# kobigurk/phase2-bn254

Measured on AMD Instinct MI355X. Metric: BN254 G1 MSM throughput (Mscalar-mul/s) at 2^26 points, higher is better.
Workload: dtype u32x8 (256-bit Montgomery limbs)

## Files before the change

### phase2-bn254_amd/csrc/msm_common.hpp

```cpp
#pragma once
#include <stdint.h>

namespace zk {

constexpr uint32_t SIGN_BIT = 0x80000000u;

struct MsmGeom {
  uint32_t c;
  uint32_t W;
  uint32_t nb;
  uint8_t width[64];
  uint8_t shift[64];
  uint32_t rmul;
  uint32_t rshift;
};

constexpr uint32_t MSM_SIZE_BINS = 4096;
constexpr uint32_t PART_THREADS = 1024;
constexpr uint32_t PART_MAX_ST = 16384;
constexpr uint32_t PART_MAX_EB = PART_MAX_ST / PART_THREADS;
constexpr uint32_t PART_LO_MAX = 12;
constexpr uint32_t PART_EC = 32;
constexpr uint32_t PART_LDS_A = 76 * 1024;
constexpr uint32_t PART_LDS_MAX = 160 * 1024 - 512;
constexpr uint32_t KEY_NONE_MASK = 0x00ffffffu;

struct PartGeom {
  uint32_t lo_bits;
  uint32_t nbin;
  uint32_t st;
  uint32_t n_st;
  uint32_t n_chunk;
  uint32_t rows_per_chunk;
};

constexpr uint32_t BIG_SEG = PART_EC * PART_THREADS;

struct BigPlan {
  uint32_t n_big;
  uint32_t total_seg;
};

constexpr uint32_t MSM_HEAVY_BLOCKS = 65536;
constexpr uint32_t MSM_HEAVY_SEG = 4096;
constexpr uint32_t MSM_HEAVY_LANES = 64;
constexpr uint32_t MSM_PAIR_MAX_BUCKETS = 3u << 17;

constexpr uint32_t MSM_FINAL_MAX = 1024;
constexpr uint32_t MSM_TREE_SLICE = 512;
// ... 5 lines not shown
```

### phase2-bn254_amd/csrc/msm_partition.hip

```cpp
#include "msm_partition.hpp"

#include <map>
#include <mutex>
#include <vector>

#include "field.hpp"
#include "msm_digits.hpp"

namespace zk {

std::atomic<int> g_msm_inflight[16];

namespace {


template <class In, class Out>
__device__ __forceinline__ uint32_t block_scan_1024(uint32_t len, uint32_t* scratch, In value, Out out) {
  constexpr uint32_t PER = 4;
  const uint32_t tid = threadIdx.x, lane = tid & 63u, wv = tid >> 6;
  uint32_t v[PER], sum = 0;
#pragma unroll
  for (uint32_t k = 0; k < PER; ++k) {
    const uint32_t idx = tid * PER + k;
    v[k] = idx < len ? value(idx) : 0u;
// ... 80 lines not shown
        for (int l = 0; l < 8; ++l) s[l] = f.l[l];
      }
      const uint32_t any = s[0] | s[1] | s[2] | s[3] | s[4] | s[5] | s[6] | s[7];
      if (active && (s[7] >> 30)) {
        atomicMin(err_scalar, (unsigned long long)(i + i_bias));
        active = false;
      }
      if (!active || any == 0) {
        for (uint32_t wl = 0; wl < WL; ++wl) keys[(uint64_t)wl * kstride + i] = G.nb;
        continue;
      }
      msm_scalar_digits<RM>(s, G, w_lo, w_hi < G.W ? w_hi : G.W, [&](uint32_t w, uint32_t d, uint32_t neg) {
        if (w >= w_lo && w < w_hi) {
          const uint32_t wl = w - w_lo;
          keys[(uint64_t)wl * kstride + i] = d ? ((d - 1) | neg) : G.nb;
          if (d) {
            const uint32_t cell = wl * P.nbin + ((d - 1) >> P.lo_bits);
            atomicAdd(&lh[cell >> 1], 1u << (16u * (cell & 1u)));
          }
        }
      });
    }
    __syncthreads();
    uint32_t* row = reinterpret_cast<uint32_t*>(tile_hist) + (uint64_t)st * nword;
    for (uint32_t t = threadIdx.x; t < nword; t += PART_THREADS) row[t] = lh[t];
    __syncthreads();
  }
}

template <uint32_t RM>
__global__ void __launch_bounds__(256) msm_digits_plain_kernel(const uint32_t* __restrict__ scalars, uint64_t n, const uint32_t* __restrict__ density,
                                                              MsmGeom G, uint32_t w_lo, uint32_t w_hi, int scalars_mont, uint64_t kstride,
// ... 31 lines not shown
  msm_scalar_digits<RM>(s, G, w_lo, w_hi < G.W ? w_hi : G.W, [&](uint32_t w, uint32_t d, uint32_t neg) {
    if (w >= w_lo && w < w_hi) keys[(uint64_t)(w - w_lo) * kstride + i] = d ? ((d - 1) | neg) : G.nb;
  });
}

__global__ void __launch_bounds__(PART_THREADS) msm_tile_hist_kernel(const uint32_t* __restrict__ keys, uint64_t n, uint64_t kstride, uint32_t nb,
                                                                     uint32_t WL, PartGeom P, uint16_t* __restrict__ tile_hist) {
  extern __shared__ __attribute__((aligned(16))) unsigned char smem[];
  uint32_t* lh = reinterpret_cast<uint32_t*>(smem);
  const uint32_t st = blockIdx.x % P.n_st, wl = blockIdx.x / P.n_st;
  const uint64_t i0 = (uint64_t)st * P.st;
  const uint32_t cnt = (uint32_t)(n - i0 < P.st ? n - i0 : P.st);
  for (uint32_t t = threadIdx.x; t < P.nbin; t += PART_THREADS) lh[t] = 0;
  __syncthreads();
  const uint32_t* kp = keys + (uint64_t)wl * kstride + i0;
  for (uint32_t idx = 4u * threadIdx.x; idx < cnt; idx += 4u * PART_THREADS) {
    uint32_t v[4] = {nb, nb, nb, nb};
    if (idx + 4 <= cnt) {
      const uint4 q = *reinterpret_cast<const uint4*>(kp + idx);
      v[0] = q.x; v[1] = q.y; v[2] = q.z; v[3] = q.w;
    } else {
      for (uint32_t e = 0; e < 4; ++e)
        if (idx + e < cnt) v[e] = kp[idx + e];
    }
#pragma unroll
    for (uint32_t e = 0; e < 4; ++e) {
      const uint32_t b = v[e] & KEY_NONE_MASK;
      if (b < nb) atomicAdd(&lh[b >> P.lo_bits], 1u);
    }
  }
  __syncthreads();
  const uint32_t ncell = WL * P.nbin, stride = (ncell + 1u) & ~1u;
  uint16_t* row = tile_hist + (uint64_t)st * stride + (uint64_t)wl * P.nbin;
  for (uint32_t t = threadIdx.x; t < P.nbin; t += PART_THREADS) row[t] = (uint16_t)lh[t];
}

__global__ void __launch_bounds__(256) msm_colsum_kernel(const uint16_t* __restrict__ tile_hist, PartGeom P, uint32_t ncell,
                                                        uint32_t* __restrict__ csum) {
  const uint32_t col = blockIdx.x * blockDim.x + threadIdx.x, chunk = blockIdx.y;
  if (col >= ncell) return;
  const uint32_t stride = (ncell + 1u) & ~1u;
  const uint32_t r0 = chunk * P.rows_per_chunk, r1 = r0 + P.rows_per_chunk < P.n_st ? r0 + P.rows_per_chunk : P.n_st;
  uint32_t s = 0;
#pragma unroll 8
  for (uint32_t r = r0; r < r1; ++r) s += tile_hist[(uint64_t)r * stride + col];
// ... 3 lines not shown
__global__ void __launch_bounds__(256) msm_colscan_kernel(uint32_t* __restrict__ csum, PartGeom P, uint32_t ncell, uint32_t* __restrict__ total) {
  const uint32_t col = blockIdx.x * blockDim.x + threadIdx.x;
  if (col >= ncell) return;
  uint32_t run = 0;
  for (uint32_t ch = 0; ch < P.n_chunk; ++ch) {
    const uint32_t v = csum[(uint64_t)ch * ncell + col];
    csum[(uint64_t)ch * ncell + col] = run;
    run += v;
  }
  total[col] = run;
}

__global__ void __launch_bounds__(PART_THREADS) msm_binscan_kernel(const uint32_t* __restrict__ total, PartGeom P, uint32_t ncell, uint32_t nb,
                                                                   uint32_t* __restrict__ bin_start, uint32_t* __restrict__ out_start) {
  __shared__ uint32_t scratch[32];
  auto padded = [&](uint32_t col) {
    const uint32_t bin = col % P.nbin;
    const uint32_t nf = ((bin + 1) << P.lo_bits) <= nb ? 1u << P.lo_bits : nb - (bin << P.lo_bits);
    return (total[col] + 3u * nf + 3u) & ~3u;
  };
  const uint32_t t0 = block_scan_long(ncell, scratch, [&](uint32_t c) { return total[c]; }, [&](uint32_t c, uint32_t ex) { bin_start[c] = ex; });
  const uint32_t t1 = block_scan_long(ncell, scratch, padded, [&](uint32_t c, uint32_t ex) { out_start[c] = ex; });
  if (threadIdx.x == 0) {
    bin_start[ncell] = t0;
    out_start[ncell] = t1;
  }
}

__global__ void __launch_bounds__(256) msm_tileoff_kernel(const uint16_t* __restrict__ tile_hist, const uint32_t* __restrict__ cbase,
                                                         const uint32_t* __restrict__ bin_start, PartGeom P, uint32_t ncell,
                                                         uint32_t* __restrict__ tile_off) {
  const uint32_t col = blockIdx.x * blockDim.x + threadIdx.x, chunk = blockIdx.y;
  if (col >= ncell) return;
  const uint32_t stride = (ncell + 1u) & ~1u;
  const uint32_t r0 = chunk * P.rows_per_chunk, r1 = r0 + P.rows_per_chunk < P.n_st ? r0 + P.rows_per_chunk : P.n_st;
// ... 23 lines not shown
    const uint32_t b = blockIdx.x;
    if (per != 0 && b < body * WL) {
      const uint32_t x = b % xcds, j = b / xcds;
      st = x * per + j % per;
      wl = j / per;
    } else {
      const uint32_t r = b - body * WL, rem = P.n_st - body;
      st = body + r % rem;
      wl = r / rem;
    }
  }
  const uint64_t i0 = (uint64_t)st * P.st;
  const uint32_t cnt = (uint32_t)(n - i0 < P.st ? n - i0 : P.st);
  for (uint32_t t = threadIdx.x; t < P.nbin; t += PART_THREADS) loff[t] = 0;
  __syncthreads();
  uint32_t key[PART_MAX_EB], rank[PART_MAX_EB];
  const uint32_t* kp = keys + (uint64_t)wl * kstride + i0;
  const bool wide = true;
#pragma unroll
  for (uint32_t k4 = 0; k4 < PART_MAX_EB / 4; ++k4) {
    const uint32_t idx = 4u * (k4 * PART_THREADS + threadIdx.x);
    uint32_t v[4] = {nb, nb, nb, nb};
    if (wide && idx + 4 <= cnt) {
      const uint4 q = *reinterpret_cast<const uint4*>(kp + idx);
      v[0] = q.x; v[1] = q.y; v[2] = q.z; v[3] = q.w;
    } else {
#pragma unroll
      for (uint32_t e = 0; e < 4; ++e)
        if (idx + e < cnt) v[e] = kp[idx + e];
    }
#pragma unroll
    for (uint32_t e = 0; e < 4; ++e) {
      key[4 * k4 + e] = v[e];
      rank[4 * k4 + e] = 0;
      const uint32_t b = v[e] & KEY_NONE_MASK;
      if (b < nb) rank[4 * k4 + e] = atomicAdd(&loff[b >> P.lo_bits], 1u);
    }
  }
  __syncthreads();
  const uint32_t* toff = tile_off + ((uint64_t)st * WL + wl) * P.nbin;
  const uint32_t total = block_scan_1024(P.nbin, scratch, [&](uint32_t x) { return loff[x]; },
                                         [&](uint32_t x, uint32_t ex) { loff[x] = ex; delta[x] = toff[x] - ex; });
  __syncthreads();
#pragma unroll
  for (uint32_t k4 = 0; k4 < PART_MAX_EB / 4; ++k4) {
#pragma unroll
    for (uint32_t e = 0; e < 4; ++e) {
      const uint32_t k = 4 * k4 + e;
      const uint32_t idx = 4u * (k4 * PART_THREADS + threadIdx.x) + e;
      const uint32_t b = key[k] & KEY_NONE_MASK;
      if (idx < cnt && b < nb) {
        uint64_t i = i0 + idx, tw = 0;
        if (flat_stride != 0) {
          tw = i / flat_stride;
          i -= tw * flat_stride;
          tw *= table_stride;
        }
        uint64_t bi = base_offset + i;
        if (density != nullptr) {
          const uint32_t wd = density[i >> 5];
          bi = base_offset + dprefix[i >> 5] + __popc(wd & ((1u << (i & 31)) - 1u));
        }
        bi += tw;
        staging[loff[b >> P.lo_bits] + rank[k]] = make_uint2(key[k], (uint32_t)bi);
      }
    }
  }
  __syncthreads();
  for (uint32_t p = threadIdx.x; p < total; p += PART_THREADS) {
    const uint2 e = staging[p];
    pairs[(uint64_t)(p + delta[(e.x & KEY_NONE_MASK) >> P.lo_bits])] = e;
  }
}

__global__ void __launch_bounds__(PART_THREADS) msm_bucket_kernel(const uint2* __restrict__ pairs, const uint32_t* __restrict__ bin_start,
                                                                  const uint32_t* __restrict__ out_start, uint32_t nb, PartGeom P,
                                                                  uint32_t stage_cap, uint32_t* __restrict__ first, uint32_t* __restrict__ last,
                                                                  uint32_t* __restrict__ vals) {
  extern __shared__ __attribute__((aligned(16))) unsigned char smem[];
  const uint32_t nfmax = 1u << P.lo_bits;
  const uint32_t nfl = nfmax < 4 ? 4 : nfmax;
  uint32_t* hist = reinterpret_cast<uint32_t*>(smem);
  uint32_t* start = hist + nfl;
  uint32_t* scratch = start + nfl;
  uint32_t* staging = scratch + 32;
  const uint32_t col = blockIdx.x, wl = col / P.nbin, bin = col % P.nbin;
  const uint32_t beg = bin_start[col], cnt = bin_start[col + 1] - beg;
  const uint32_t ob = out_start[col];
  const uint32_t nf = (bin + 1) << P.lo_bits <= nb ? nfmax : nb - (bin << P.lo_bits);
  const uint32_t fmask = nfmax - 1u;
  for (uint32_t t = threadIdx.x; t < nfmax; t += PART_THREADS) hist[t] = 0;
  __syncthreads();
  if (cnt > PART_EC * PART_THREADS) return;
  uint32_t val[PART_EC], fr[PART_EC];
#pragma unroll
  for (uint32_t k = 0; k < PART_EC; ++k) {
    const uint32_t idx = k * PART_THREADS + threadIdx.x;
    val[k] = 0;
    fr[k] = 0;
    if (idx < cnt) {
      const uint2 e = pairs[(uint64_t)beg + idx];
      const uint32_t f = e.x & fmask;
      val[k] = e.y | (e.x & SIGN_BIT);
      fr[k] = f | (atomicAdd(&hist[f], 1u) << PART_LO_MAX);
    }
  }
  __syncthreads();
  const uint32_t padded = block_scan_1024(nf, scratch, [&](uint32_t x) { return (hist[x] + 3u) & ~3u; },
                                          [&](uint32_t x, uint32_t ex) { start[x] = ex; });
  __syncthreads();
  const uint32_t id0 = wl * nb + (bin << P.lo_bits);
  for (uint32_t t = threadIdx.x; t < nf; t += PART_THREADS) {
    first[id0 + t] = ob + start[t];
    last[id0 + t] = ob + start[t] + hist[t];
  }
  if (padded <= stage_cap) {
#pragma unroll
    for (uint32_t k = 0; k < PART_EC; ++k) {
      const uint32_t idx = k * PART_THREADS + threadIdx.x;
      if (idx < cnt) staging[start[fr[k] & ((1u << PART_LO_MAX) - 1u)] + (fr[k] >> PART_LO_MAX)] = val[k];
    }
    __syncthreads();
    uint4* dst = reinterpret_cast<uint4*>(vals + ob);
    const uint4* src = reinterpret_cast<const uint4*>(staging);
    for (uint32_t q = threadIdx.x; q < padded / 4; q += PART_THREADS) dst[q] = src[q];
  } else {
// ... 24 lines not shown

__global__ void __launch_bounds__(PART_THREADS) msm_scan_small_kernel(const uint16_t* __restrict__ tile_hist, PartGeom P, uint32_t ncell, uint32_t nb,
                                                                      uint32_t* __restrict__ col_total, uint32_t* __restrict__ bin_start,
                                                                      uint32_t* __restrict__ out_start, uint32_t* __restrict__ tile_off,
                                                                      uint32_t* __restrict__ size_hist, uint32_t* __restrict__ big_col,
                                                                      uint32_t* __restrict__ big_seg_off, BigPlan* __restrict__ plan) {
  __shared__ uint32_t scratch[32];
  const uint32_t stride = (ncell + 1u) & ~1u;
  for (uint32_t t = threadIdx.x; t < MSM_SIZE_BINS; t += PART_THREADS) size_hist[t] = 0;
  for (uint32_t col = threadIdx.x; col < ncell; col += PART_THREADS) {
    uint32_t s = 0;
    for (uint32_t r = 0; r < P.n_st; ++r) s += tile_hist[(uint64_t)r * stride + col];
    col_total[col] = s;
  }
  __syncthreads();
  auto padded = [&](uint32_t col) {
    const uint32_t bin = col % P.nbin;
    const uint32_t nf = ((bin + 1) << P.lo_bits) <= nb ? 1u << P.lo_bits : nb - (bin << P.lo_bits);
    return (col_total[col] + 3u * nf + 3u) & ~3u;
  };
  const uint32_t t0 = block_scan_long(ncell, scratch, [&](uint32_t c) { return col_total[c]; }, [&](uint32_t c, uint32_t ex) { bin_start[c] = ex; });
  const uint32_t t1 = block_scan_long(ncell, scratch, padded, [&](uint32_t c, uint32_t ex) { out_start[c] = ex; });
  if (threadIdx.x == 0) {
    bin_start[ncell] = t0;
    out_start[ncell] = t1;
  }
  __syncthreads();
  for (uint32_t col = threadIdx.x; col < ncell; col += PART_THREADS) {
    uint32_t run = bin_start[col];
    for (uint32_t r = 0; r < P.n_st; ++r) {
      tile_off[(uint64_t)r * ncell + col] = run;
      run += tile_hist[(uint64_t)r * stride + col];
    }
  }
  auto cnt_of = [&](uint32_t col) { return bin_start[col + 1] - bin_start[col]; };
// ... 19 lines not shown
  }
  *col = big_col[lo];
  *seg = b - big_seg_off[lo];
  return true;
}

__global__ void __launch_bounds__(PART_THREADS) msm_bigbin_count_kernel(const uint2* __restrict__ pairs, const uint32_t* __restrict__ bin_start,
                                                                        const BigPlan* __restrict__ plan, const uint32_t* __restrict__ big_col,
                                                                        const uint32_t* __restrict__ big_seg_off, uint32_t nb, PartGeom P,
                                                                        uint32_t* __restrict__ gcnt) {
  extern __shared__ __attribute__((aligned(16))) unsigned char smem[];
  uint32_t* hist = reinterpret_cast<uint32_t*>(smem);
  for (uint32_t b = blockIdx.x;; b += gridDim.x) {
    uint32_t col, seg;
    if (!bigbin_locate(plan, big_col, big_seg_off, b, &col, &seg)) return;
    const uint32_t nfmax = 1u << P.lo_bits, fmask = nfmax - 1u;
    const uint32_t wl = col / P.nbin, bin = col % P.nbin;
    const uint32_t beg = bin_start[col] + seg * BIG_SEG, end = bin_start[col + 1];
    const uint32_t cnt = end - beg < BIG_SEG ? end - beg : BIG_SEG;
    for (uint32_t t = threadIdx.x; t < nfmax; t += PART_THREADS) hist[t] = 0;
    __syncthreads();
    for (uint32_t idx = threadIdx.x; idx < cnt; idx += PART_THREADS) atomicAdd(&hist[pairs[(uint64_t)beg + idx].x & fmask], 1u);
    __syncthreads();
    const uint32_t id0 = wl * nb + (bin << P.lo_bits);
    for (uint32_t t = threadIdx.x; t < nfmax; t += PART_THREADS)
      if (hist[t]) atomicAdd(&gcnt[id0 + t], hist[t]);
    __syncthreads();
  }
}

__global__ void __launch_bounds__(PART_THREADS) msm_bigbin_place_kernel(const uint2* __restrict__ pairs, const uint32_t* __restrict__ bin_start,
                                                                        const uint32_t* __restrict__ out_start, const BigPlan* __restrict__ plan,
                                                                        const uint32_t* __restrict__ big_col, const uint32_t* __restrict__ big_seg_off,
                                                                        uint32_t nb, PartGeom P, int staged, const uint32_t* __restrict__ gcnt,
                                                                        uint32_t* __restrict__ gcur, uint32_t* __restrict__ first,
                                                                        uint32_t* __restrict__ last, uint32_t* __restrict__ vals) {
  extern __shared__ __attribute__((aligned(16))) unsigned char smem[];
  for (uint32_t blk = blockIdx.x;; blk += gridDim.x) {
  uint32_t col, seg;
  if (!bigbin_locate(plan, big_col, big_seg_off, blk, &col, &seg)) return;
  const uint32_t nfmax = 1u << P.lo_bits, fmask = nfmax - 1u;
  const uint32_t nfl = nfmax < 4 ? 4 : nfmax;
  uint32_t* hist = reinterpret_cast<uint32_t*>(smem);
  uint32_t* start = hist + nfl;
  uint32_t* scratch = start + nfl;
  uint32_t* lstart = scratch + 32;
  uint32_t* llen = lstart + nfl;
  uint32_t* staging = llen + nfl;
  const uint32_t wl = col / P.nbin, bin = col % P.nbin;
  const uint32_t beg = bin_start[col] + seg * BIG_SEG, end = bin_start[col + 1];
  const uint32_t cnt = end - beg < BIG_SEG ? end - beg : BIG_SEG;
  const uint32_t ob = out_start[col];
  const uint32_t nf = (bin + 1) << P.lo_bits <= nb ? nfmax : nb - (bin << P.lo_bits);
  const uint32_t id0 = wl * nb + (bin << P.lo_bits);
  for (uint32_t t = threadIdx.x; t < nfmax; t += PART_THREADS) hist[t] = 0;
  __syncthreads();
  uint32_t val[PART_EC], fr[PART_EC];
#pragma unroll
  for (uint32_t k = 0; k < PART_EC; ++k) {
    const uint32_t idx = k * PART_THREADS + threadIdx.x;
    val[k] = 0;
    fr[k] = 0;
    if (idx < cnt) {
      const uint2 e = pairs[(uint64_t)beg + idx];
      const uint32_t f = e.x & fmask;
      val[k] = e.y | (e.x & SIGN_BIT);
      fr[k] = f | (atomicAdd(&hist[f], 1u) << PART_LO_MAX);
    }
  }
  __syncthreads();
  block_scan_1024(nf, scratch, [&](uint32_t x) { return (gcnt[id0 + x] + 3u) & ~3u; }, [&](uint32_t x, uint32_t ex) { start[x] = ex; });
  if (staged) block_scan_1024(nf, scratch, [&](uint32_t x) { return hist[x]; }, [&](uint32_t x, uint32_t ex) { lstart[x] = ex; });
  __syncthreads();
  for (uint32_t t = threadIdx.x; t < nf; t += PART_THREADS) {
    if (seg == 0) {
      first[id0 + t] = ob + start[t];
      last[id0 + t] = ob + start[t] + gcnt[id0 + t];
    }
    const uint32_t mine = hist[t];
    if (staged) llen[t] = mine;
// ... 136 lines not shown
  for (const void* fn : fns) {
    hipError_t e = hipFuncSetAttribute(fn, hipFuncAttributeMaxDynamicSharedMemorySize, 160 * 1024);
    if (e != hipSuccess) {
      std::fprintf(stderr, "[mi355zk] hipFuncSetAttribute(partition kernel, 160 KiB LDS) failed: %s\n", hipGetErrorString(e));
      rc = ZK_ERR_DEVICE;
    }
  }
  g_part_cfg[dev] = rc;
  return rc;
}

int msm_checkpoint(const MsmPartCall& A, const char* what, const ChunkPlan& C) {
  if (!A.knobs.debug) return 0;
  const MsmPlan& P = A.plan;
  ZK_HIP(hipStreamSynchronize(A.st));
  std::fprintf(stderr, "[mi355zk] msm<%d> n=%llu chunk@%llu+%llu c=%u W=%u buckets=%u levels=%u part(lo=%u nbin=%u st=%u): %s done\n", A.group,
               (unsigned long long)A.n, (unsigned long long)C.lo, (unsigned long long)C.n, P.G.c, P.WL, P.n_buckets, P.n_levels, C.P.lo_bits, C.P.nbin,
               C.P.st, what);
  return 0;
}

void msm_order_by_size(const uint32_t* first, const uint32_t* last, uint32_t n_buckets, uint32_t* hist, uint32_t* order, uint32_t* sizes_sorted,
                       hipStream_t st) {
  uint32_t hb = (n_buckets + 4095) / 4096;
  hipLaunchKernelGGL(msm_size_hist_kernel, dim3(hb < 1024 ? hb : 1024), dim3(1024), 0, st, first, last, n_buckets, hist);
  hipLaunchKernelGGL(msm_size_scan_kernel, dim3(1), dim3(1024), 0, st, hist);
  hipLaunchKernelGGL(msm_size_scatter_kernel, dim3((n_buckets + 1024 * MSM_SCATTER_PER - 1) / (1024 * MSM_SCATTER_PER)), dim3(1024), 0, st, first,
                     last, n_buckets, hist, order, sizes_sorted);
}

void launch_heavy_plan(hipStream_t st, const uint32_t* sizes_sorted, uint32_t hb, uint32_t heavy, uint32_t seg, uint32_t* item_off) {
  hipLaunchKernelGGL(msm_heavy_plan_kernel, dim3(1), dim3(1024), 0, st, sizes_sorted, hb, heavy, seg, item_off);
}
// ... 56 lines not shown
    hipLaunchKernelGGL(msm_tileoff_kernel, dim3((ncell + 255) / 256, PG.n_chunk), dim3(256), 0, st, W.tile_hist, W.csum, W.bin_start, PG, ncell, W.tile_off);
  }
  ZK_HIP(hipGetLastError());
  prof_end(S.scan, st);
  prof_begin(S.scatter, st);
  hipLaunchKernelGGL(msm_scatter_kernel, dim3(PG.n_st * WL), dim3(PART_THREADS), (size_t)(2 * ((PG.nbin + 3u) & ~3u) + 32) * 4 + (size_t)PG.st * 8, st,
                     W.keys, C.np, P.tmode ? C.np : kstride, boff, dens, dpre, G.nb, WL, PG, A.knobs.part_xcds, W.tile_off, W.pairs, P.tmode ? kstride : 0ull,
                     A.table_stride);
  ZK_HIP(hipGetLastError());
  prof_end(S.scatter, st);
  if (msm_checkpoint(A, "scatter", C)) return ZK_ERR_DEVICE;
  prof_begin(S.bucket, st);
  {
    const uint32_t nfl = (1u << PG.lo_bits) < 4 ? 4 : (1u << PG.lo_bits);
    const size_t fixed = (size_t)(2 * nfl + 32) * 4;
    uint64_t want = (uint64_t)(C.np / PG.nbin) * 5 / 4 + 3ull * nfl + 4096;
    const uint64_t cap_max = (PART_LDS_MAX - fixed) / 4;
    if (want > cap_max) want = cap_max;
    if (want > (uint64_t)PART_EC * PART_THREADS + 3ull * nfl) want = (uint64_t)PART_EC * PART_THREADS + 3ull * nfl;
    const uint32_t stage_cap = (uint32_t)want & ~3u;
    hipLaunchKernelGGL(msm_bucket_kernel, dim3(ncell), dim3(PART_THREADS), fixed + (size_t)stage_cap * 4, st, W.pairs, W.bin_start, W.out_start, G.nb, PG,
                       stage_cap, W.first, W.last, W.vals_b);
    if (C.np > BIG_SEG) {
      const uint32_t max_seg = (uint32_t)(2 * (C.m / BIG_SEG) + 2);
      if (!C.small_scan) hipLaunchKernelGGL(msm_bigbin_plan_kernel, dim3(1), dim3(PART_THREADS), 0, st, W.bin_start, ncell, W.big_col, W.big_seg, W.big_plan);
      int n_cu = 256;
      (void)hipDeviceGetAttribute(&n_cu, hipDeviceAttributeMultiprocessorCount, A.dev);
      const uint32_t big_grid = max_seg < 2u * (uint32_t)n_cu ? max_seg : 2u * (uint32_t)n_cu;
      const uint32_t place_grid = max_seg < (uint32_t)n_cu ? max_seg : (uint32_t)n_cu;
      hipLaunchKernelGGL(msm_bigbin_count_kernel, dim3(big_grid), dim3(PART_THREADS), (size_t)nfl * 4, st, W.pairs, W.bin_start, W.big_plan, W.big_col, W.big_seg,
                         G.nb, PG, W.gcnt);
// ... 52 lines not shown
```

### phase2-bn254_amd/csrc/msm_plan.hpp

```cpp
#pragma once
#include <algorithm>
#include <cmath>
#include <cstdio>
#include <cstdlib>
#include <vector>

#include "host_util.hpp"
#include "msm_common.hpp"

namespace zk {

struct MsmKnobs {
  int msm_c = 0;
  uint32_t radix_m = 0, radix_s = 0;
  bool radix_off = false;
  int table_c = 0;
  int part_lo = -1, part_st = 0;
  bool no_tail2d = false;
  bool no_small_scan = false;
  bool debug = false;
  bool fused_a = false;
  uint32_t part_xcds = 8;
  bool acc_a4 = true;
  int g1_pair = -1, g2_pair = -1;
// ... 83 lines not shown

inline MsmGeom make_geom_radix(uint32_t rmul, uint32_t rshift) {
  MsmGeom G{};
  G.rmul = rmul;
  G.rshift = rshift;
  const double B = std::ldexp((double)rmul, (int)rshift);
  G.nb = (rmul << rshift) / 2;
  G.c = 1;
  while ((1u << G.c) <= G.nb) ++G.c;
  uint32_t W = 2;
  while ((W - 1) * std::log2(B) + std::log2((double)G.nb) < 254.001) ++W;
  G.W = W;
  return G;
}

inline double geom_cost(double W, double nbk, double field_bits, uint64_t n, double top_values) {
  double cost = W * ((10.0 + 0.7 * std::ceil(field_bits / 8.0)) * (double)n + 45.0 * nbk);
  double lanes = W * nbk;
  if (lanes < 131072.0) cost *= (1.0 + 0.5 * (131072.0 / lanes - 1.0));
  const double mean = (double)n / nbk;
  const double heavy = std::max(64.0, 2.0 * mean + 16.0);
  const double top_len = (double)n / top_values;
  if (top_len > heavy) cost += 1.2e7;
  else if (top_len > 2.0 * mean + 16.0) cost += (top_len - (2.0 * mean + 16.0)) * 5e5;
  return cost;
}

inline MsmGeom choose_geom(uint64_t n, int group, uint32_t wgroups, const MsmKnobs& K) {
  if (K.radix_m && wgroups == 1) return make_geom_radix(K.radix_m, K.radix_s);
  if (K.msm_c >= 2 && K.msm_c <= 24 && wgroups == 1) return make_geom((uint32_t)K.msm_c);
  if (wgroups == 1 && n < (1ull << 20)) {
    uint32_t lg = 0;
    while ((1ull << lg) < n) ++lg;
    uint32_t c = lg <= 10 ? 10u : lg <= 12 ? 11u : lg == 13 ? 12u : lg <= 15 ? 13u : lg <= 17 ? 15u : 16u;
    if (group == 2) c = lg <= 10 ? 10u : lg == 11 ? 11u : lg <= 15 ? 12u : lg <= 17 ? 14u : lg == 18 ? 15u : 16u;
    return make_geom(c);
  }
  uint32_t best_c = 0;
  double best = 1e300;
  for (uint32_t c = 4; c <= 24; ++c) {
    double W = std::ceil((254.0 + 1.0) / c);
    if ((uint32_t)W % wgroups) continue;
    const MsmGeom Gc = make_geom(c);
    double cost = geom_cost(W, std::ldexp(1.0, (int)c - 1), c, n, std::ldexp(1.0, (int)Gc.width[Gc.W - 1]));
    if (cost < best) { best = cost; best_c = c; }
  }
  MsmGeom G{};
  if (best_c) G = make_geom(best_c);
  if (K.radix_off && best_c) return G;
  for (uint32_t rmul = 3; rmul <= 15; rmul += 2)
    for (uint32_t rshift = 4; rshift <= 22; ++rshift) {
      MsmGeom R = make_geom_radix(rmul, rshift);
      if (R.W > 64 || R.c > 24 || R.W % wgroups) continue;
      const double top_values = std::exp2(254.0 - (R.W - 1.0) * std::log2(std::ldexp((double)rmul, (int)rshift)));
      double cost = geom_cost(R.W, R.nb, R.c, n, top_values);
      if (cost < 0.985 * best) { best = cost / 0.985; G = R; }
    }
  return G;
}

inline uint32_t table_window_bits(uint64_t n_bases, int group, const MsmKnobs& K) {
  if (K.table_c >= 4 && K.table_c <= 24) return (uint32_t)K.table_c;
  uint32_t lg = 0;
  while ((1ull << lg) < n_bases) ++lg;
  if (group == 2) return lg <= 18 ? 17u : lg == 19 ? 19u : 20u;
  return lg <= 16 ? 17u : lg <= 22 ? 20u : 22u;
}

inline PartGeom choose_part(uint64_t n, uint32_t WL, uint32_t nb, const MsmKnobs& K) {
  PartGeom P{};
  uint32_t lo_cap = 0;
  while ((1u << lo_cap) < nb && lo_cap < PART_LO_MAX) ++lo_cap;
  auto nbin_of = [&](uint32_t lo) { return (uint32_t)(((uint64_t)nb + (1ull << lo) - 1) >> lo); };
  auto fits_lds = [&](uint32_t lo, uint64_t budget) { return (uint64_t)WL * nbin_of(lo) * 2 <= budget && nbin_of(lo) <= 4 * PART_THREADS; };
  auto fits = [&](uint32_t lo) { return fits_lds(lo, 2 * PART_LDS_A); };
  auto pop = [&](uint32_t lo) { return (uint64_t)n * (1ull << lo) / nb; };
  uint32_t lo = lo_cap;
  const uint64_t pop_target = 12288;
  const uint64_t pop_cap = (uint64_t)PART_EC * PART_THREADS * 85 / 100;
  while (lo > 0 && pop(lo) > pop_target && fits_lds(lo - 1, PART_LDS_A)) --lo;
  while (lo > 0 && pop(lo) > pop_cap && fits(lo - 1)) --lo;
  while (!fits(lo) && lo < PART_LO_MAX) ++lo;
  if (K.part_lo >= 0 && K.part_lo <= (int)lo_cap && fits((uint32_t)K.part_lo)) lo = (uint32_t)K.part_lo;
  P.lo_bits = lo;
  P.nbin = nbin_of(lo);
  uint32_t st = PART_MAX_ST;
  while (st > PART_THREADS && (n / st) * WL < 256) st >>= 1;
  if (K.part_st >= (int)PART_THREADS && K.part_st <= (int)PART_MAX_ST && K.part_st % (int)PART_THREADS == 0) st = (uint32_t)K.part_st;
  while (st > PART_THREADS && (uint64_t)st * 8 + (uint64_t)P.nbin * 8 + 256 > PART_LDS_MAX) st -= PART_THREADS;
  if ((uint64_t)st * 8 + (uint64_t)P.nbin * 8 + 256 > PART_LDS_MAX) st = 0;
  P.st = st;
  P.n_st = (uint32_t)((n + st - 1) / st);
  P.rows_per_chunk = P.n_st > 64 ? (P.n_st + 63) / 64 : 1;
  P.n_chunk = (P.n_st + P.rows_per_chunk - 1) / P.rows_per_chunk;
  return P;
}


struct MsmRequest {
  int group = 1;
  uint64_t n = 0;
  uint64_t base_offset = 0;
  uint32_t wgroups = 1, wgroup = 0;
  uint32_t n_chunks = 1;
  const uint64_t* cuts = nullptr;
  bool two_sets = false;
  uint64_t table_stride = 0;
  uint32_t table_c = 0;
};

struct ChunkPlan {
  uint64_t lo, n, m, np;
  PartGeom P;
  uint32_t ncell, heavy, heavy_seg, hb, max_items;
  bool small_scan;
  uint32_t split_t, split_hb;
};

struct MsmLayout {
  size_t keys, pairs, tile_hist, tile_off, csum, total, bin_start, out_start;
  size_t gcnt, gcur, big_col, big_seg, big_plan;
  size_t first, last, hist, sizes_b, ids_b, item_off, seg_sums, buckets, partA, partS;
  size_t rc;
  size_t wsums;
  size_t err;
  size_t sumtmp;
  size_t total_bytes;
  size_t back_bytes() const { return (err - wsums) + 16; }
};
// ... 34 lines not shown
  const uint32_t n_chunks = R.n_chunks;
  const uint64_t* cuts = R.cuts ? R.cuts : whole;
  if (n_chunks == 0 || (R.cuts == nullptr && n_chunks != 1) || cuts[0] != 0 || cuts[n_chunks] != n) return ZK_ERR_BAD_ARGS;
  if (n_chunks > 1 && R.two_sets) return ZK_ERR_BAD_ARGS;
  uint64_t n_max = 0;
  for (uint32_t c = 0; c < n_chunks; ++c) {
    if (cuts[c + 1] <= cuts[c] || (c > 0 && (cuts[c] & 31))) return ZK_ERR_BAD_ARGS;
    if (cuts[c + 1] - cuts[c] > n_max) n_max = cuts[c + 1] - cuts[c];
  }
  const MsmGeom G = P.G = tmode ? make_geom(R.table_c) : choose_geom(n, R.group, R.wgroups, K);
  if (G.W == 0 || G.W % R.wgroups) return ZK_ERR_BAD_ARGS;
  const uint32_t WD = P.WD = G.W / R.wgroups;
  P.w_lo = R.wgroup * WD;
  P.w_hi = P.w_lo + WD;
  const uint32_t WL = P.WL = tmode ? 1u : WD;
  if (tmode && (uint64_t)G.W * R.table_stride > 0x7fffffffull) return ZK_ERR_BAD_ARGS;
  const uint64_t m_max = P.m_max = tmode ? ((n_max + 3) & ~3ull) * WD : n_max * WL;
  if (m_max > 0xfffffff0ull) return ZK_ERR_BAD_ARGS;
  const uint32_t n_buckets = P.n_buckets = WL * G.nb;
  uint32_t final_cnt = G.nb, n_levels = 0;
  auto tail_fits = [&](uint32_t cnt) { return !K.no_tail2d && g1 && (uint64_t)cnt * WL <= (1ull << 17) && cnt >= (1u << 15) && cnt <= (1u << 18); };
  while (final_cnt > K.final_max && n_levels < MSM_MAX_LEVELS) {
    if (tail_fits(final_cnt)) break;
    uint32_t logl = (uint64_t)final_cnt * WL >= (1ull << 20) ? 3 : 2;
    if (K.logl[n_levels]) logl = K.logl[n_levels];
    P.lvl_cnt[n_levels] = final_cnt;
    P.lvl_logl[n_levels] = logl;
    P.lvl_chunks[n_levels] = (final_cnt + (1u << logl) - 1) >> logl;
    P.total_chunks += P.lvl_chunks[n_levels];
    final_cnt = P.lvl_chunks[n_levels];
// ... 9 lines not shown
    P.cols_log = (lg + 1) / 2;
  }
  const uint32_t t_cols = P.t_cols = tail2d ? 1u << P.cols_log : final_cnt, t_rows = P.t_rows = tail2d ? (final_cnt + t_cols - 1) / t_cols : 0;
  while ((1u << P.final_bits) <= t_cols - 1 + final_off) ++P.final_bits;
  while (t_rows > 1 && (1u << P.row_bits) <= t_rows - 1) ++P.row_bits;

  P.chunks.resize(n_chunks);
  uint64_t keys_cap = 0, tile_hist_b = 0, tile_off_b = 0, csum_b = 0;
  uint32_t ncell_max = 0, hb_max = 0, items_max = 0;
  for (uint32_t c = 0; c < n_chunks; ++c) {
    ChunkPlan& C = P.chunks[c];
    C.lo = cuts[c];
    C.n = cuts[c + 1] - cuts[c];
    C.np = tmode ? ((C.n + 3) & ~3ull) * WD : C.n;
    C.m = C.np * WL;
    C.P = choose_part(C.np, WL, G.nb, K);
    if (C.P.st == 0) return ZK_ERR_BAD_ARGS;
    C.ncell = WL * C.P.nbin;
    C.small_scan = !K.no_small_scan && (uint64_t)C.P.n_st * C.ncell <= (1u << 16);
    const uint64_t vals_cap = C.m + 3ull * n_buckets + 4ull * C.ncell + 4;
    if (vals_cap > 0xfffffff0ull) return ZK_ERR_BAD_ARGS;
    keys_cap = std::max(keys_cap, vals_cap);
    tile_hist_b = std::max<uint64_t>(tile_hist_b, (uint64_t)C.P.n_st * ((C.ncell + 1) & ~1u) * 2);
    tile_off_b = std::max<uint64_t>(tile_off_b, (uint64_t)C.P.n_st * C.ncell * 4);
    csum_b = std::max<uint64_t>(csum_b, (uint64_t)C.P.n_chunk * C.ncell * 4);
    ncell_max = std::max(ncell_max, C.ncell);
    const uint64_t mean_len = C.m / n_buckets + 1;
    uint64_t heavy64 = mean_len * 8 + 1024;
    const uint64_t heavy_cap = (C.m >> 17) > 64 ? (C.m >> 17) : 64;
    if (heavy64 > heavy_cap) heavy64 = heavy_cap;
    if (heavy64 < 2 * mean_len + 16) heavy64 = 2 * mean_len + 16;
    C.heavy = (uint32_t)(heavy64 > 0xffffffffull ? 0xffffffffull : heavy64);
    C.heavy_seg = 128;
// ... 65 lines not shown
```

Measured before the change: 1011.

## Use finer partition bins for the sparsely populated top window

The top MSM window holds only a small range of digit values, so with uniform coarse bins its points pile into a few overloaded bins. The change adds per-window bin widths (a split point and a smaller lo width) for the last window, so its populated range spreads over more bins. Digits above the reachable range are skipped, and their bucket first/last entries are zeroed directly. This targets load imbalance and oversized bins in the partition and bucket kernels, at the cost of extra index arithmetic per key and a larger PartGeom kernel argument.

Result: no change. 1012 (median of 2 runs) (+0.1%).

```diff
diff --git a/phase2-bn254_amd/csrc/msm_common.hpp b/phase2-bn254_amd/csrc/msm_common.hpp
--- a/phase2-bn254_amd/csrc/msm_common.hpp
+++ b/phase2-bn254_amd/csrc/msm_common.hpp
@@ -25,6 +25,8 @@
 constexpr uint32_t PART_LDS_MAX = 160 * 1024 - 512;
 constexpr uint32_t KEY_NONE_MASK = 0x00ffffffu;
 
+constexpr uint32_t PART_MAX_W = 72;
+
 struct PartGeom {
   uint32_t lo_bits;
   uint32_t nbin;
@@ -32,7 +34,27 @@
   uint32_t n_st;
   uint32_t n_chunk;
   uint32_t rows_per_chunk;
+  uint16_t split_w[PART_MAX_W];
+  uint8_t lo_w[PART_MAX_W];
+
+  constexpr uint32_t edge(uint32_t wl) const { return (uint32_t)split_w[wl] << lo_w[wl]; }
+  constexpr uint32_t part_end(uint32_t wl, uint32_t nb) const {
+    const uint64_t e = (uint64_t)edge(wl) + ((uint64_t)(nbin - split_w[wl]) << lo_bits);
+    return e < nb ? (uint32_t)e : nb;
+  }
 };
+
+constexpr uint32_t part_bin_of(uint32_t b, uint32_t lo_w, uint32_t split, uint32_t lo_bits) {
+  const uint32_t edge = split << lo_w;
+  return b < edge ? b >> lo_w : split + ((b - edge) >> lo_bits);
+}
+struct PartCell { uint32_t wl, base, bits, count; };
+constexpr PartCell part_cell(const PartGeom& P, uint32_t col, uint32_t nb) {
+  const uint32_t wl = col / P.nbin, bin = col % P.nbin, lo_w = P.lo_w[wl], split = P.split_w[wl];
+  const uint32_t base = bin < split ? bin << lo_w : (split << lo_w) + ((bin - split) << P.lo_bits), bits = bin < split ? lo_w : P.lo_bits;
+  const uint32_t end = P.part_end(wl, nb);
+  return {wl, base, bits, base >= end ? 0u : end - base < (1u << bits) ? end - base : 1u << bits};
+}
 
 constexpr uint32_t BIG_SEG = PART_EC * PART_THREADS;
 
diff --git a/phase2-bn254_amd/csrc/msm_partition.hip b/phase2-bn254_amd/csrc/msm_partition.hip
--- a/phase2-bn254_amd/csrc/msm_partition.hip
+++ b/phase2-bn254_amd/csrc/msm_partition.hip
@@ -118,8 +118,8 @@
         if (w >= w_lo && w < w_hi) {
           const uint32_t wl = w - w_lo;
           keys[(uint64_t)wl * kstride + i] = d ? ((d - 1) | neg) : G.nb;
-          if (d) {
-            const uint32_t cell = wl * P.nbin + ((d - 1) >> P.lo_bits);
+          if (d && d - 1 < P.part_end(wl, G.nb)) {
+            const uint32_t cell = wl * P.nbin + part_bin_of(d - 1, P.lo_w[wl], P.split_w[wl], P.lo_bits);
             atomicAdd(&lh[cell >> 1], 1u << (16u * (cell & 1u)));
           }
         }
@@ -181,21 +181,26 @@
   for (uint32_t t = threadIdx.x; t < P.nbin; t += PART_THREADS) lh[t] = 0;
   __syncthreads();
   const uint32_t* kp = keys + (uint64_t)wl * kstride + i0;
-  for (uint32_t idx = 4u * threadIdx.x; idx < cnt; idx += 4u * PART_THREADS) {
-    uint32_t v[4] = {nb, nb, nb, nb};
-    if (idx + 4 <= cnt) {
-      const uint4 q = *reinterpret_cast<const uint4*>(kp + idx);
-      v[0] = q.x; v[1] = q.y; v[2] = q.z; v[3] = q.w;
-    } else {
-      for (uint32_t e = 0; e < 4; ++e)
-        if (idx + e < cnt) v[e] = kp[idx + e];
-    }
-#pragma unroll
-    for (uint32_t e = 0; e < 4; ++e) {
-      const uint32_t b = v[e] & KEY_NONE_MASK;
-      if (b < nb) atomicAdd(&lh[b >> P.lo_bits], 1u);
-    }
-  }
+  const uint32_t lo_w = P.lo_w[wl], split = P.split_w[wl], end = P.part_end(wl, nb);
+  auto count = [&](auto bin_of) {
+    for (uint32_t idx = 4u * threadIdx.x; idx < cnt; idx += 4u * PART_THREADS) {
+      uint32_t v[4] = {nb, nb, nb, nb};
+      if (idx + 4 <= cnt) {
+        const uint4 q = *reinterpret_cast<const uint4*>(kp + idx);
+        v[0] = q.x; v[1] = q.y; v[2] = q.z; v[3] = q.w;
+      } else {
+        for (uint32_t e = 0; e < 4; ++e)
+          if (idx + e < cnt) v[e] = kp[idx + e];
+      }
+#pragma unroll
+      for (uint32_t e = 0; e < 4; ++e) {
+        const uint32_t b = v[e] & KEY_NONE_MASK;
+        if (b < end) atomicAdd(&lh[bin_of(b)], 1u);
+      }
+    }
+  };
+  if (lo_w == P.lo_bits) count([&](uint32_t b) { return b >> P.lo_bits; });
+  else count([&](uint32_t b) { return part_bin_of(b, lo_w, split, P.lo_bits); });
   __syncthreads();
   const uint32_t ncell = WL * P.nbin, stride = (ncell + 1u) & ~1u;
   uint16_t* row = tile_hist + (uint64_t)st * stride + (uint64_t)wl * P.nbin;
@@ -229,11 +234,7 @@
 __global__ void __launch_bounds__(PART_THREADS) msm_binscan_kernel(const uint32_t* __restrict__ total, PartGeom P, uint32_t ncell, uint32_t nb,
                                                                    uint32_t* __restrict__ bin_start, uint32_t* __restrict__ out_start) {
   __shared__ uint32_t scratch[32];
-  auto padded = [&](uint32_t col) {
-    const uint32_t bin = col % P.nbin;
-    const uint32_t nf = ((bin + 1) << P.lo_bits) <= nb ? 1u << P.lo_bits : nb - (bin << P.lo_bits);
-    return (total[col] + 3u * nf + 3u) & ~3u;
-  };
+  auto padded = [&](uint32_t col) { return (total[col] + 3u * part_cell(P, col, nb).count + 3u) & ~3u; };
   const uint32_t t0 = block_scan_long(ncell, scratch, [&](uint32_t c) { return total[c]; }, [&](uint32_t c, uint32_t ex) { bin_start[c] = ex; });
   const uint32_t t1 = block_scan_long(ncell, scratch, padded, [&](uint32_t c, uint32_t ex) { out_start[c] = ex; });
   if (threadIdx.x == 0) {
@@ -287,63 +288,68 @@
   const uint32_t cnt = (uint32_t)(n - i0 < P.st ? n - i0 : P.st);
   for (uint32_t t = threadIdx.x; t < P.nbin; t += PART_THREADS) loff[t] = 0;
   __syncthreads();
-  uint32_t key[PART_MAX_EB], rank[PART_MAX_EB];
   const uint32_t* kp = keys + (uint64_t)wl * kstride + i0;
-  const bool wide = true;
-#pragma unroll
-  for (uint32_t k4 = 0; k4 < PART_MAX_EB / 4; ++k4) {
-    const uint32_t idx = 4u * (k4 * PART_THREADS + threadIdx.x);
-    uint32_t v[4] = {nb, nb, nb, nb};
-    if (wide && idx + 4 <= cnt) {
-      const uint4 q = *reinterpret_cast<const uint4*>(kp + idx);
-      v[0] = q.x; v[1] = q.y; v[2] = q.z; v[3] = q.w;
-    } else {
-#pragma unroll
-      for (uint32_t e = 0; e < 4; ++e)
-        if (idx + e < cnt) v[e] = kp[idx + e];
-    }
-#pragma unroll
-    for (uint32_t e = 0; e < 4; ++e) {
-      key[4 * k4 + e] = v[e];
-      rank[4 * k4 + e] = 0;
-      const uint32_t b = v[e] & KEY_NONE_MASK;
-      if (b < nb) rank[4 * k4 + e] = atomicAdd(&loff[b >> P.lo_bits], 1u);
-    }
-  }
-  __syncthreads();
-  const uint32_t* toff = tile_off + ((uint64_t)st * WL + wl) * P.nbin;
-  const uint32_t total = block_scan_1024(P.nbin, scratch, [&](uint32_t x) { return loff[x]; },
-                                         [&](uint32_t x, uint32_t ex) { loff[x] = ex; delta[x] = toff[x] - ex; });
-  __syncthreads();
-#pragma unroll
-  for (uint32_t k4 = 0; k4 < PART_MAX_EB / 4; ++k4) {
-#pragma unroll
-    for (uint32_t e = 0; e < 4; ++e) {
-      const uint32_t k = 4 * k4 + e;
-      const uint32_t idx = 4u * (k4 * PART_THREADS + threadIdx.x) + e;
-      const uint32_t b = key[k] & KEY_NONE_MASK;
-      if (idx < cnt && b < nb) {
-        uint64_t i = i0 + idx, tw = 0;
-        if (flat_stride != 0) {
-          tw = i / flat_stride;
-          i -= tw * flat_stride;
-          tw *= table_stride;
+  const uint32_t lo_w = P.lo_w[wl], split = P.split_w[wl], end = P.part_end(wl, nb);
+  auto run = [&](auto bin_of) {
+    uint32_t key[PART_MAX_EB], rank[PART_MAX_EB];
+    const bool wide = true;
+#pragma unroll
+    for (uint32_t k4 = 0; k4 < PART_MAX_EB / 4; ++k4) {
+      const uint32_t idx = 4u * (k4 * PART_THREADS + threadIdx.x);
+      uint32_t v[4] = {nb, nb, nb, nb};
+      if (wide && idx + 4 <= cnt) {
+        const uint4 q = *reinterpret_cast<const uint4*>(kp + idx);
+        v[0] = q.x; v[1] = q.y; v[2] = q.z; v[3] = q.w;
+      } else {
+#pragma unroll
+        for (uint32_t e = 0; e < 4; ++e)
+          if (idx + e < cnt) v[e] = kp[idx + e];
+      }
+#pragma unroll
+      for (uint32_t e = 0; e < 4; ++e) {
+        key[4 * k4 + e] = v[e];
+        rank[4 * k4 + e] = 0;
+        const uint32_t b = v[e] & KEY_NONE_MASK;
+        if (b < end) rank[4 * k4 + e] = atomicAdd(&loff[bin_of(b)], 1u);
+      }
+    }
+    __syncthreads();
+    const uint32_t* toff = tile_off + ((uint64_t)st * WL + wl) * P.nbin;
+    const uint32_t total = block_scan_1024(P.nbin, scratch, [&](uint32_t x) { return loff[x]; },
+                                           [&](uint32_t x, uint32_t ex) { loff[x] = ex; delta[x] = toff[x] - ex; });
+    __syncthreads();
+#pragma unroll
+    for (uint32_t k4 = 0; k4 < PART_MAX_EB / 4; ++k4) {
+#pragma unroll
+      for (uint32_t e = 0; e < 4; ++e) {
+        const uint32_t k = 4 * k4 + e;
+        const uint32_t idx = 4u * (k4 * PART_THREADS + threadIdx.x) + e;
+        const uint32_t b = key[k] & KEY_NONE_MASK;
+        if (idx < cnt && b < end) {
+          uint64_t i = i0 + idx, tw = 0;
+          if (flat_stride != 0) {
+            tw = i / flat_stride;
+            i -= tw * flat_stride;
+            tw *= table_stride;
+          }
+          uint64_t bi = base_offset + i;
+          if (density != nullptr) {
+            const uint32_t wd = density[i >> 5];
+            bi = base_offset + dprefix[i >> 5] + __popc(wd & ((1u << (i & 31)) - 1u));
+          }
+          bi += tw;
+          staging[loff[bin_of(b)] + rank[k]] = make_uint2(key[k], (uint32_t)bi);
         }
-        uint64_t bi = base_offset + i;
-        if (density != nullptr) {
-          const uint32_t wd = density[i >> 5];
-          bi = base_offset + dprefix[i >> 5] + __popc(wd & ((1u << (i & 31)) - 1u));
-        }
-        bi += tw;
-        staging[loff[b >> P.lo_bits] + rank[k]] = make_uint2(key[k], (uint32_t)bi);
-      }
-    }
-  }
-  __syncthreads();
-  for (uint32_t p = threadIdx.x; p < total; p += PART_THREADS) {
-    const uint2 e = staging[p];
-    pairs[(uint64_t)(p + delta[(e.x & KEY_NONE_MASK) >> P.lo_bits])] = e;
-  }
+      }
+    }
+    __syncthreads();
+    for (uint32_t p = threadIdx.x; p < total; p += PART_THREADS) {
+      const uint2 e = staging[p];
+      pairs[(uint64_t)(p + delta[bin_of(e.x & KEY_NONE_MASK)])] = e;
+    }
+  };
+  if (lo_w == P.lo_bits) run([&](uint32_t b) { return b >> P.lo_bits; });
+  else run([&](uint32_t b) { return part_bin_of(b, lo_w, split, P.lo_bits); });
 }
 
 __global__ void __launch_bounds__(PART_THREADS) msm_bucket_kernel(const uint2* __restrict__ pairs, const uint32_t* __restrict__ bin_start,
@@ -351,18 +357,22 @@
                                                                   uint32_t stage_cap, uint32_t* __restrict__ first, uint32_t* __restrict__ last,
                                                                   uint32_t* __restrict__ vals) {
   extern __shared__ __attribute__((aligned(16))) unsigned char smem[];
-  const uint32_t nfmax = 1u << P.lo_bits;
-  const uint32_t nfl = nfmax < 4 ? 4 : nfmax;
+  const uint32_t nfl = (1u << P.lo_bits) < 4 ? 4 : 1u << P.lo_bits;
   uint32_t* hist = reinterpret_cast<uint32_t*>(smem);
   uint32_t* start = hist + nfl;
   uint32_t* scratch = start + nfl;
   uint32_t* staging = scratch + 32;
-  const uint32_t col = blockIdx.x, wl = col / P.nbin, bin = col % P.nbin;
+  const uint32_t col = blockIdx.x;
+  const PartCell cell = part_cell(P, col, nb);
+  const uint32_t wl = cell.wl, nf = cell.count;
   const uint32_t beg = bin_start[col], cnt = bin_start[col + 1] - beg;
   const uint32_t ob = out_start[col];
-  const uint32_t nf = (bin + 1) << P.lo_bits <= nb ? nfmax : nb - (bin << P.lo_bits);
-  const uint32_t fmask = nfmax - 1u;
-  for (uint32_t t = threadIdx.x; t < nfmax; t += PART_THREADS) hist[t] = 0;
+  const uint32_t end = P.part_end(wl, nb);
+  if (end < nb) {
+    const uint32_t per = (nb - end + P.nbin - 1) / P.nbin, t0 = end + (col % P.nbin) * per;
+    for (uint32_t t = t0 + threadIdx.x; t < t0 + per && t < nb; t += PART_THREADS) first[wl * nb + t] = last[wl * nb + t] = 0;
+  }
+  for (uint32_t t = threadIdx.x; t < nf; t += PART_THREADS) hist[t] = 0;
   __syncthreads();
   if (cnt > PART_EC * PART_THREADS) return;
   uint32_t val[PART_EC], fr[PART_EC];
@@ -373,7 +383,7 @@
     fr[k] = 0;
     if (idx < cnt) {
       const uint2 e = pairs[(uint64_t)beg + idx];
-      const uint32_t f = e.x & fmask;
+      const uint32_t f = (e.x & KEY_NONE_MASK) - cell.base;
       val[k] = e.y | (e.x & SIGN_BIT);
       fr[k] = f | (atomicAdd(&hist[f], 1u) << PART_LO_MAX);
     }
@@ -382,7 +392,7 @@
   const uint32_t padded = block_scan_1024(nf, scratch, [&](uint32_t x) { return (hist[x] + 3u) & ~3u; },
                                           [&](uint32_t x, uint32_t ex) { start[x] = ex; });
   __syncthreads();
-  const uint32_t id0 = wl * nb + (bin << P.lo_bits);
+  const uint32_t id0 = wl * nb + cell.base;
   for (uint32_t t = threadIdx.x; t < nf; t += PART_THREADS) {
     first[id0 + t] = ob + start[t];
     last[id0 + t] = ob + start[t] + hist[t];
@@ -437,11 +447,7 @@
     col_total[col] = s;
   }
   __syncthreads();
-  auto padded = [&](uint32_t col) {
-    const uint32_t bin = col % P.nbin;
-    const uint32_t nf = ((bin + 1) << P.lo_bits) <= nb ? 1u << P.lo_bits : nb - (bin << P.lo_bits);
-    return (col_total[col] + 3u * nf + 3u) & ~3u;
-  };
+  auto padded = [&](uint32_t col) { return (col_total[col] + 3u * part_cell(P, col, nb).count + 3u) & ~3u; };
   const uint32_t t0 = block_scan_long(ncell, scratch, [&](uint32_t c) { return col_total[c]; }, [&](uint32_t c, uint32_t ex) { bin_start[c] = ex; });
   const uint32_t t1 = block_scan_long(ncell, scratch, padded, [&](uint32_t c, uint32_t ex) { out_start[c] = ex; });
   if (threadIdx.x == 0) {
@@ -491,16 +497,15 @@
   for (uint32_t b = blockIdx.x;; b += gridDim.x) {
     uint32_t col, seg;
     if (!bigbin_locate(plan, big_col, big_seg_off, b, &col, &seg)) return;
-    const uint32_t nfmax = 1u << P.lo_bits, fmask = nfmax - 1u;
-    const uint32_t wl = col / P.nbin, bin = col % P.nbin;
+    const PartCell cell = part_cell(P, col, nb);
     const uint32_t beg = bin_start[col] + seg * BIG_SEG, end = bin_start[col + 1];
     const uint32_t cnt = end - beg < BIG_SEG ? end - beg : BIG_SEG;
-    for (uint32_t t = threadIdx.x; t < nfmax; t += PART_THREADS) hist[t] = 0;
-    __syncthreads();
-    for (uint32_t idx = threadIdx.x; idx < cnt; idx += PART_THREADS) atomicAdd(&hist[pairs[(uint64_t)beg + idx].x & fmask], 1u);
-    __syncthreads();
-    const uint32_t id0 = wl * nb + (bin << P.lo_bits);
-    for (uint32_t t = threadIdx.x; t < nfmax; t += PART_THREADS)
+    for (uint32_t t = threadIdx.x; t < cell.count; t += PART_THREADS) hist[t] = 0;
+    __syncthreads();
+    for (uint32_t idx = threadIdx.x; idx < cnt; idx += PART_THREADS) atomicAdd(&hist[(pairs[(uint64_t)beg + idx].x & KEY_NONE_MASK) - cell.base], 1u);
+    __syncthreads();
+    const uint32_t id0 = cell.wl * nb + cell.base;
+    for (uint32_t t = threadIdx.x; t < cell.count; t += PART_THREADS)
       if (hist[t]) atomicAdd(&gcnt[id0 + t], hist[t]);
     __syncthreads();
   }
@@ -516,21 +521,20 @@
   for (uint32_t blk = blockIdx.x;; blk += gridDim.x) {
   uint32_t col, seg;
   if (!bigbin_locate(plan, big_col, big_seg_off, blk, &col, &seg)) return;
-  const uint32_t nfmax = 1u << P.lo_bits, fmask = nfmax - 1u;
-  const uint32_t nfl = nfmax < 4 ? 4 : nfmax;
+  const uint32_t nfl = (1u << P.lo_bits) < 4 ? 4 : 1u << P.lo_bits;
   uint32_t* hist = reinterpret_cast<uint32_t*>(smem);
   uint32_t* start = hist + nfl;
   uint32_t* scratch = start + nfl;
   uint32_t* lstart = scratch + 32;
   uint32_t* llen = lstart + nfl;
   uint32_t* staging = llen + nfl;
-  const uint32_t wl = col / P.nbin, bin = col % P.nbin;
+  const PartCell cell = part_cell(P, col, nb);
   const uint32_t beg = bin_start[col] + seg * BIG_SEG, end = bin_start[col + 1];
   const uint32_t cnt = end - beg < BIG_SEG ? end - beg : BIG_SEG;
   const uint32_t ob = out_start[col];
-  const uint32_t nf = (bin + 1) << P.lo_bits <= nb ? nfmax : nb - (bin << P.lo_bits);
-  const uint32_t id0 = wl * nb + (bin << P.lo_bits);
-  for (uint32_t t = threadIdx.x; t < nfmax; t += PART_THREADS) hist[t] = 0;
+  const uint32_t nf = cell.count;
+  const uint32_t id0 = cell.wl * nb + cell.base;
+  for (uint32_t t = threadIdx.x; t < nf; t += PART_THREADS) hist[t] = 0;
   __syncthreads();
   uint32_t val[PART_EC], fr[PART_EC];
 #pragma unroll
@@ -540,7 +544,7 @@
     fr[k] = 0;
     if (idx < cnt) {
       const uint2 e = pairs[(uint64_t)beg + idx];
-      const uint32_t f = e.x & fmask;
+      const uint32_t f = (e.x & KEY_NONE_MASK) - cell.base;
       val[k] = e.y | (e.x & SIGN_BIT);
       fr[k] = f | (atomicAdd(&hist[f], 1u) << PART_LO_MAX);
     }
@@ -707,9 +711,9 @@
   if (!A.knobs.debug) return 0;
   const MsmPlan& P = A.plan;
   ZK_HIP(hipStreamSynchronize(A.st));
-  std::fprintf(stderr, "[mi355zk] msm<%d> n=%llu chunk@%llu+%llu c=%u W=%u buckets=%u levels=%u part(lo=%u nbin=%u st=%u): %s done\n", A.group,
+  std::fprintf(stderr, "[mi355zk] msm<%d> n=%llu chunk@%llu+%llu c=%u W=%u buckets=%u levels=%u part(lo=%u nbin=%u st=%u; last window lo=%u x %u bins): %s done\n", A.group,
                (unsigned long long)A.n, (unsigned long long)C.lo, (unsigned long long)C.n, P.G.c, P.WL, P.n_buckets, P.n_levels, C.P.lo_bits, C.P.nbin,
-               C.P.st, what);
+               C.P.st, (unsigned)C.P.lo_w[P.WL - 1], (unsigned)C.P.split_w[P.WL - 1], what);
   return 0;
 }
 
@@ -796,7 +800,7 @@
   {
     const uint32_t nfl = (1u << PG.lo_bits) < 4 ? 4 : (1u << PG.lo_bits);
     const size_t fixed = (size_t)(2 * nfl + 32) * 4;
-    uint64_t want = (uint64_t)(C.np / PG.nbin) * 5 / 4 + 3ull * nfl + 4096;
+    uint64_t want = (uint64_t)C.bin_pop * 5 / 4 + 3ull * nfl + 4096;
     const uint64_t cap_max = (PART_LDS_MAX - fixed) / 4;
     if (want > cap_max) want = cap_max;
     if (want > (uint64_t)PART_EC * PART_THREADS + 3ull * nfl) want = (uint64_t)PART_EC * PART_THREADS + 3ull * nfl;
diff --git a/phase2-bn254_amd/csrc/msm_plan.hpp b/phase2-bn254_amd/csrc/msm_plan.hpp
--- a/phase2-bn254_amd/csrc/msm_plan.hpp
+++ b/phase2-bn254_amd/csrc/msm_plan.hpp
@@ -121,6 +121,16 @@
   return G;
 }
 
+struct TopValues { double expect, bound; };
+inline TopValues top_window_values(const MsmGeom& G) {
+  if (G.rmul == 1) {
+    const double v = std::ldexp(1.0, (int)G.width[G.W - 1]);
+    return {v, v};
+  }
+  const double lg_top = (G.W - 1.0) * std::log2(std::ldexp((double)G.rmul, (int)G.rshift));
+  return {std::exp2(253.59669135500215  - lg_top), std::exp2(254.0 - lg_top)};
+}
+
 inline double geom_cost(double W, double nbk, double field_bits, uint64_t n, double top_values) {
   double cost = W * ((10.0 + 0.7 * std::ceil(field_bits / 8.0)) * (double)n + 45.0 * nbk);
   double lanes = W * nbk;
@@ -149,7 +159,7 @@
     double W = std::ceil((254.0 + 1.0) / c);
     if ((uint32_t)W % wgroups) continue;
     const MsmGeom Gc = make_geom(c);
-    double cost = geom_cost(W, std::ldexp(1.0, (int)c - 1), c, n, std::ldexp(1.0, (int)Gc.width[Gc.W - 1]));
+    double cost = geom_cost(W, std::ldexp(1.0, (int)c - 1), c, n, top_window_values(Gc).bound);
     if (cost < best) { best = cost; best_c = c; }
   }
   MsmGeom G{};
@@ -159,8 +169,7 @@
     for (uint32_t rshift = 4; rshift <= 22; ++rshift) {
       MsmGeom R = make_geom_radix(rmul, rshift);
       if (R.W > 64 || R.c > 24 || R.W % wgroups) continue;
-      const double top_values = std::exp2(254.0 - (R.W - 1.0) * std::log2(std::ldexp((double)rmul, (int)rshift)));
-      double cost = geom_cost(R.W, R.nb, R.c, n, top_values);
+      double cost = geom_cost(R.W, R.nb, R.c, n, top_window_values(R).bound);
       if (cost < 0.985 * best) { best = cost / 0.985; G = R; }
     }
   return G;
@@ -174,7 +183,7 @@
   return lg <= 16 ? 17u : lg <= 22 ? 20u : 22u;
 }
 
-inline PartGeom choose_part(uint64_t n, uint32_t WL, uint32_t nb, const MsmKnobs& K) {
+inline PartGeom choose_part(uint64_t n, uint32_t WL, uint32_t nb, const TopValues* top, const MsmKnobs& K) {
   PartGeom P{};
   uint32_t lo_cap = 0;
   while ((1u << lo_cap) < nb && lo_cap < PART_LO_MAX) ++lo_cap;
@@ -191,6 +200,19 @@
   if (K.part_lo >= 0 && K.part_lo <= (int)lo_cap && fits((uint32_t)K.part_lo)) lo = (uint32_t)K.part_lo;
   P.lo_bits = lo;
   P.nbin = nbin_of(lo);
+  for (uint32_t wl = 0; wl < WL && wl < PART_MAX_W; ++wl) P.lo_w[wl] = (uint8_t)lo, P.split_w[wl] = (uint16_t)P.nbin;
+  if (top != nullptr && WL >= 1 && WL <= PART_MAX_W && top->bound + 2.0 < (double)nb) {
+    const uint32_t values = (uint32_t)std::ceil(top->expect), cover = (uint32_t)top->bound + 2;
+    auto split_of = [&](uint32_t lw) { return (uint32_t)(((uint64_t)values + (1ull << lw) - 1) >> lw); };
+    auto pop_top = [&](uint32_t lw) { return (uint64_t)n * (1ull << lw) / values; };
+    auto fits_top = [&](uint32_t lw) {
+      const uint64_t s = split_of(lw);
+      return s <= P.nbin && (s << lw) + ((P.nbin - s) << lo) >= cover;
+    };
+    uint32_t lw = lo;
+    while (lw > 0 && pop_top(lw) > pop_cap && fits_top(lw - 1)) --lw;
+    if (lw < lo) P.lo_w[WL - 1] = (uint8_t)lw, P.split_w[WL - 1] = (uint16_t)split_of(lw);
+  }
   uint32_t st = PART_MAX_ST;
   while (st > PART_THREADS && (n / st) * WL < 256) st >>= 1;
   if (K.part_st >= (int)PART_THREADS && K.part_st <= (int)PART_MAX_ST && K.part_st % (int)PART_THREADS == 0) st = (uint32_t)K.part_st;
@@ -220,6 +242,7 @@
   uint64_t lo, n, m, np;
   PartGeom P;
   uint32_t ncell, heavy, heavy_seg, hb, max_items;
+  uint32_t bin_pop;
   bool small_scan;
   uint32_t split_t, split_hb;
 };
@@ -284,6 +307,7 @@
   P.w_lo = R.wgroup * WD;
   P.w_hi = P.w_lo + WD;
   const uint32_t WL = P.WL = tmode ? 1u : WD;
+  if (WL > PART_MAX_W) return ZK_ERR_BAD_ARGS;
   if (tmode && (uint64_t)G.W * R.table_stride > 0x7fffffffull) return ZK_ERR_BAD_ARGS;
   const uint64_t m_max = P.m_max = tmode ? ((n_max + 3) & ~3ull) * WD : n_max * WL;
   if (m_max > 0xfffffff0ull) return ZK_ERR_BAD_ARGS;
@@ -323,9 +347,12 @@
     C.n = cuts[c + 1] - cuts[c];
     C.np = tmode ? ((C.n + 3) & ~3ull) * WD : C.n;
     C.m = C.np * WL;
-    C.P = choose_part(C.np, WL, G.nb, K);
+    const TopValues top = top_window_values(G);
+    C.P = choose_part(C.np, WL, G.nb, !tmode && P.w_hi == G.W ? &top : nullptr, K);
     if (C.P.st == 0) return ZK_ERR_BAD_ARGS;
     C.ncell = WL * C.P.nbin;
+    C.bin_pop = 0;
+    for (uint32_t wl = 0; wl < WL; ++wl) C.bin_pop = std::max(C.bin_pop, (uint32_t)(C.np / C.P.split_w[wl]));
     C.small_scan = !K.no_small_scan && (uint64_t)C.P.n_st * C.ncell <= (1u << 16);
     const uint64_t vals_cap = C.m + 3ull * n_buckets + 4ull * C.ncell + 4;
     if (vals_cap > 0xfffffff0ull) return ZK_ERR_BAD_ARGS;
```
